# tsbertalan/openmg

Measured on AMD Instinct MI355X. Metric: V-cycles/sec, 3-D 7-point Poisson 256^3, higher is better.
Workload: dtype f64

## Files before the change

openmg_amd/csrc/plane.hip:

```cpp
#include <algorithm>
#include <array>
#include <atomic>
#include <cmath>
#include <cstring>
#include <map>
#include <mutex>
#include <thread>
#include <type_traits>

#include "common.h"
#include "peer_wait.h"
#include "sine_cube16.h"

#if defined(OMG_PLANE_STAMPS) || defined(OMG_PLANE_DBGARGS)
#define OMG_PLANE_DBG_ON 1
#endif

namespace omg {
namespace {

#ifndef PLANE_STORE_AUX
#define PLANE_STORE_AUX 2
#endif
typedef unsigned v2u __attribute__((ext_vector_type(2)));
typedef unsigned v4u __attribute__((ext_vector_type(4)));
typedef int v2i __attribute__((ext_vector_type(2)));

__device__ __forceinline__ double madd(double v, double x, double acc) { return fma(v, x, acc); }
__device__ __forceinline__ float madd(float v, float x, float acc) { return fmaf(v, x, acc); }

template <typename V>
struct P2 {
    V x, y;
};
template <typename V> struct VecOf;
template <> struct VecOf<double> {
    typedef double type __attribute__((ext_vector_type(2)));
    typedef type gtype __attribute__((aligned(8)));
};
template <> struct VecOf<float> {
    typedef float type __attribute__((ext_vector_type(2)));
    typedef type gtype __attribute__((aligned(4)));
};

__device__ __forceinline__ P2<double> bload2(__amdgpu_buffer_rsrc_t rs, int off, double) {
    const v4u q = __builtin_amdgcn_raw_buffer_load_b128(rs, off, 0, 0);
    return {__builtin_bit_cast(double, v2u{q.x, q.y}), __builtin_bit_cast(double, v2u{q.z, q.w})};
}
__device__ __forceinline__ P2<float> bload2(__amdgpu_buffer_rsrc_t rs, int off, float) {
    typedef float v2f __attribute__((ext_vector_type(2)));
    const v2f q = __builtin_bit_cast(v2f, __builtin_amdgcn_raw_buffer_load_b64(rs, off, 0, 0));
    return {q.x, q.y};
}
__device__ __forceinline__ double bload1(__amdgpu_buffer_rsrc_t rs, int off, double) {
    return __builtin_bit_cast(double, __builtin_amdgcn_raw_buffer_load_b64(rs, off, 0, 0));
}
__device__ __forceinline__ float bload1(__amdgpu_buffer_rsrc_t rs, int off, float) {
    return __builtin_bit_cast(float, __builtin_amdgcn_raw_buffer_load_b32(rs, off, 0, 0));
}
template <typename V>
__device__ __forceinline__ P2<V> lds_pair(const V *p) {
    const typename VecOf<V>::type q = *reinterpret_cast<const typename VecOf<V>::type *>(p);
    return {q.x, q.y};
}
template <typename V>
__device__ __forceinline__ void lds_put(V *p, const P2<V> &v) {
    typename VecOf<V>::type q;
    q.x = v.x;
    q.y = v.y;
    *reinterpret_cast<typename VecOf<V>::type *>(p) = q;
}
template <int AUX = PLANE_STORE_AUX>
__device__ __forceinline__ void bstore2(__amdgpu_buffer_rsrc_t rs, int off, const P2<double> &v, bool both) {
    if (both) {
        const v2u lo = __builtin_bit_cast(v2u, v.x), hi = __builtin_bit_cast(v2u, v.y);
        __builtin_amdgcn_raw_buffer_store_b128(v4u{lo.x, lo.y, hi.x, hi.y}, rs, off, 0, AUX);
    } else {
        __builtin_amdgcn_raw_buffer_store_b64(__builtin_bit_cast(v2u, v.x), rs, off, 0, AUX);
    }
}
template <int AUX = 0>
__device__ __forceinline__ void bstore2(__amdgpu_buffer_rsrc_t rs, int off, const P2<float> &v, bool both) {
    if (both) {
        __builtin_amdgcn_raw_buffer_store_b64(v2u{__builtin_bit_cast(unsigned, v.x), __builtin_bit_cast(unsigned, v.y)}, rs, off, 0, AUX);
    } else {
        __builtin_amdgcn_raw_buffer_store_b32(__builtin_bit_cast(unsigned, v.x), rs, off, 0, AUX);
    }
}
template <int AUX>
__device__ __forceinline__ void bstore1(__amdgpu_buffer_rsrc_t rs, int off, double v) {
    __builtin_amdgcn_raw_buffer_store_b64(__builtin_bit_cast(v2u, v), rs, off, 0, AUX);
}
template <int AUX>
__device__ __forceinline__ void bstore1(__amdgpu_buffer_rsrc_t rs, int off, float v) {
    __builtin_amdgcn_raw_buffer_store_b32(__builtin_bit_cast(unsigned, v), rs, off, 0, AUX);
}
constexpr int PEER_PLANES = 3, PEER_CPLANES = 2;
constexpr int PEER_AUX = 1 | 16;
template <typename V>
__device__ __forceinline__ void store2(V *p, const P2<V> &v, bool both) {
    if (both) {
        typename VecOf<V>::gtype q;
        q.x = v.x;
        q.y = v.y;
        *reinterpret_cast<typename VecOf<V>::gtype *>(p) = q;
    } else {
        p[0] = v.x;
    }
}

#ifndef PLANE_LA_BIG
#define PLANE_LA_BIG 1
#endif
#ifndef PLANE_LA
#define PLANE_LA 1
#endif
#ifndef PLANE_WAVE_SYNC
#define PLANE_WAVE_SYNC 1
#endif
constexpr unsigned WAVE_SYNC_SPIN = 1u << 22;
constexpr int OOB = 0x7FFFFFF0;

template <typename V>
struct PlaneKArgs {
    const V *x_old;
    V *x_new;
    const V *b;
    unsigned vec_bytes;
    int nr;
    int hx, ny, nz;
    int z_base, z_end, kv0, kv1, kc_off;
    int TXq, TY, LZ, PX, PY, ntx, nty, ntz;
    int zc_base, zc_stride, zc_len, zc_end, part_slot0;
    int edge_wg0;
    V c0, c1, c2, c3, c4, c5, c6, w;
    V wp;
    int x_zero;
    int fast_div;
    int nxc, nyc, nzc;
    unsigned cvec_bytes, cmap_bytes;
    const int32_t *cmap;
    V *bc, *xc;
    const V *cdiag;
    int first_end;
    const V *ec;
    double *partials;
    V *peer_x[2], *peer_bc[2];
    int peer_shift, peer_cshift;
    const uint32_t *wait_flag[4];
    uint32_t wait_seq[4];
    int fused_wait;
    uint32_t *done, *peer_flag[2];
    uint32_t flag_seq, spin;
    uint32_t *status;
#ifdef OMG_PLANE_STAMPS
    unsigned long long *stamps;
#endif
#ifdef OMG_PLANE_DBG_ON
    int dbg;
#endif
};

template <typename V>
__device__ __forceinline__ V chain_head(const PlaneKArgs<V> &a, V km, V jm, V im) {
    V s = madd(a.c0, km, V(0));
    s = madd(a.c1, jm, s);
    return madd(a.c2, im, s);
}
template <typename V>
__device__ __forceinline__ V chain_tail(const PlaneKArgs<V> &a, V s, V d, V ip, V jp, V kp) {
    s = madd(a.c3, d, s);
    s = madd(a.c4, ip, s);
    s = madd(a.c5, jp, s);
    return madd(a.c6, kp, s);
}

__device__ __forceinline__ double refined_rcp(double d) {
    double r = __builtin_amdgcn_rcp(d);
    double e = fma(-d, r, 1.0);
    r = fma(r, e, r);
    e = fma(-d, r, 1.0);
    return fma(r, e, r);
}
__device__ __forceinline__ float refined_rcp(float) { return 0.0f; }
__device__ __forceinline__ bool plain_numerator(double v) {
    const unsigned e = ((unsigned)__double2hiint(v) >> 20) & 0x7ffu;
    return e - 623u <= 800u || v == 0.0;
}
__device__ __forceinline__ bool plain_numerator(float) { return false; }
template <typename V>
__device__ __forceinline__ void quotients(const V (&n)[4], V c, V r, bool fast, V (&q)[4]) {
    if (sizeof(V) == 8 && fast) {
        bool bad = false;
#pragma unroll
        for (int i = 0; i < 4; ++i) {
            const V q0 = n[i] * r;
            q[i] = madd(madd(-c, q0, n[i]), r, q0);
            bad = bad || !plain_numerator(n[i]);
        }
        if (__builtin_amdgcn_ballot_w64(bad) == 0) return;
    }
#pragma unroll
    for (int i = 0; i < 4; ++i) q[i] = n[i] / c;
}

template <typename V>
struct Inline {
    V imx, ipx, imy, ipy;
};
template <typename V>
__device__ __forceinline__ Inline<V> in_line(int rule, const P2<V> &O, V nb) {
    Inline<V> r;
    r.imx = rule ? O.x : nb;
    r.ipx = rule ? O.y : O.x;
    r.imy = rule ? O.y : O.x;
    r.ipy = rule ? nb : O.y;
    return r;
}

__device__ __forceinline__ void peer_done(uint32_t *done, uint32_t n_wg, uint32_t *const (&flag)[2], uint32_t seq) {
    __builtin_amdgcn_fence(__ATOMIC_RELEASE, "workgroup");
    __syncthreads();
    if (threadIdx.x == 0) {
        const uint32_t before = __hip_atomic_fetch_add(done, 1u, __ATOMIC_RELAXED, __HIP_MEMORY_SCOPE_AGENT);
        if (before == n_wg - 1) {
            __hip_atomic_store(done, 0u, __ATOMIC_RELAXED, __HIP_MEMORY_SCOPE_AGENT);
            for (int i = 0; i < 2; ++i)
                if (flag[i]) __hip_atomic_store(flag[i], seq, __ATOMIC_RELAXED, __HIP_MEMORY_SCOPE_SYSTEM);
        }
    }
}
__global__ void plane_wait_kernel(const uint32_t *f0, const uint32_t *f1, const uint32_t *f2, const uint32_t *f3,
                                  uint32_t s0, uint32_t s1, uint32_t s2, uint32_t s3, uint32_t *status, uint32_t spin) {
    if (threadIdx.x == 0) {
        peer_wait(f0, s0, status, spin);
        peer_wait(f1, s1, status, spin);
        peer_wait(f2, s2, status, spin);
        peer_wait(f3, s3, status, spin);
    }
}

template <typename V, int MODE, bool NORM, bool XZ, int LA, bool PEER = false, int MAXT = 512, bool FIRST = false, bool SWEEP = true, bool MIRROR = false>
__global__ __launch_bounds__(MAXT) void plane_kernel(const PlaneKArgs<V> a) {
    static_assert(!MIRROR || (MODE == 1 && !PEER && !FIRST && !XZ), "mirrored march: up passes of whole grids");
#ifdef OMG_PLANE_STAMPS
    const unsigned long long st_entry = __builtin_amdgcn_s_memtime();
#endif
    extern __shared__ __attribute__((aligned(16))) unsigned char plane_smem[];
    V *const lds = reinterpret_cast<V *>(plane_smem);
    __shared__ double s_red[8];
    __shared__ int s_step[8];
    if (threadIdx.x < 8) s_step[threadIdx.x] = 0;

    const int PX = a.PX, PY = a.PY;
    const int S = 2 * PX + 4;
    const int BUF = (2 * PY + 2) * S;
    const int t = int(threadIdx.x);
    const bool live = t < PX * PY;
    const int px = live ? t % PX : 0, py = live ? t / PX : 0;
    int L = int(blockIdx.x);
    int nwg = int(gridDim.x);
    const bool edge_wg = !PEER && a.edge_wg0 > 0 && L >= a.edge_wg0;
    if (!PEER && a.edge_wg0 > 0) {
        if (edge_wg) { L -= a.edge_wg0; nwg = 1; }
        else nwg = a.edge_wg0;
    }
    if ((nwg & 7) == 0) L = (L & 7) * (nwg >> 3) + (L >> 3);
    const int nxy = a.ntx * a.nty;
    const int tz = L / nxy, rem = L - tz * nxy;
    const int ty = rem / a.ntx, tx = rem - ty * a.ntx;
    const int z0 = edge_wg ? (tz ? a.z_end - PLANE_EDGE : a.z_base) : a.zc_base + tz * a.zc_stride;
    const int z1 = edge_wg ? z0 + PLANE_EDGE : min(a.zc_end, z0 + a.zc_len);
    const int q = tx * a.TXq + px - 1;
    const int ja = ty * a.TY + 2 * py - 4;
    const bool vx0 = live && q >= 0 && 2 * q < a.hx, vx1 = live && q >= 0 && 2 * q + 1 < a.hx;
    const bool vl[2] = {ja >= 0 && ja < a.ny, ja + 1 >= 0 && ja + 1 < a.ny};
    const bool inner = live && px >= 1 && px <= PX - 2 && py >= 2 && py <= PY - 3;
    const int ps = a.ny * a.hx;
    const int lb[2] = {ja * a.hx + 2 * q, (ja + 1) * a.hx + 2 * q};

    const __amdgpu_buffer_rsrc_t xs = __builtin_amdgcn_make_buffer_rsrc(const_cast<V *>(a.x_old), 0, a.vec_bytes, 0x00020000);
    const __amdgpu_buffer_rsrc_t bs = __builtin_amdgcn_make_buffer_rsrc(const_cast<V *>(a.b), 0, a.vec_bytes, 0x00020000);
    const __amdgpu_buffer_rsrc_t ws = __builtin_amdgcn_make_buffer_rsrc(a.x_new, 0, a.vec_bytes, 0x00020000);
    const __amdgpu_buffer_rsrc_t es = __builtin_amdgcn_make_buffer_rsrc(const_cast<V *>(MODE == 1 ? a.ec : a.cdiag), 0, a.cvec_bytes, 0x00020000);
    const __amdgpu_buffer_rsrc_t ms = __builtin_amdgcn_make_buffer_rsrc(const_cast<int32_t *>(a.cmap), 0, a.cmap_bytes, 0x00020000);

    constexpr int W = int(sizeof(V));
    const bool vcell = vl[0] && vx0;
    V c1a = ja > 0 ? a.c1 : V(0);
    V c5b = ja + 2 < a.ny ? a.c5 : V(0);
    V c2x = q > 0 ? a.c2 : V(0);
    V c4x = 2 * q + 1 < a.hx ? a.c4 : V(0);
    V c4y = 2 * q + 2 < a.hx ? a.c4 : V(0);
    unsigned lbo[2] = {vcell ? unsigned(lb[0] * W) : unsigned(OOB), vcell ? unsigned(lb[1] * W) : unsigned(OOB)};
    unsigned lso[2] = {(vcell && inner) ? unsigned(lb[0] * W) : unsigned(OOB), (vcell && inner) ? unsigned(lb[1] * W) : unsigned(OOB)};
    asm volatile("" : "+v"(c1a), "+v"(c5b), "+v"(c2x), "+v"(c4x), "+v"(c4y));
    asm volatile("" : "+v"(lbo[0]), "+v"(lbo[1]), "+v"(lso[0]), "+v"(lso[1]));
    const bool oddx = (a.hx & 1) != 0;

    auto head = [&](int l, int v, int rule, V km, V jm, V im) -> V {
        V sum = madd(a.c0, km, V(0));
        sum = madd(l == 0 ? c1a : a.c1, jm, sum);
        return madd((v == 0 && rule == 0) ? c2x : a.c2, im, sum);
    };
    auto tail = [&](int l, int v, int rule, V sum, V d, V ip, V jp, V kp) -> V {
        sum = madd(a.c3, d, sum);
        sum = madd(rule == 0 ? a.c4 : (v == 0 ? c4x : c4y), ip, sum);
        sum = madd(l == 1 ? c5b : a.c5, jp, sum);
        return madd(a.c6, kp, sum);
    };

    auto zphys = [&](int k) -> int { return MIRROR ? a.nz - 1 - k : k; };
    auto cplane = [&](int kc) -> int { return MIRROR ? (a.nz / 2 - 1 + a.kc_off) - kc : kc + a.kc_off; };
    auto plane_off = [&](int colour, int k) -> unsigned {
        return (k >= a.kv0 && k < a.kv1) ? unsigned(((colour ? a.nr : 0) + zphys(k) * ps) * W) : unsigned(OOB);
    };
    auto fetch = [&](const __amdgpu_buffer_rsrc_t &rs, int colour, int k, int l) -> P2<V> {
        unsigned po = plane_off(colour, k);
        asm volatile("" : "+s"(po));
        return bload2(rs, int(lbo[l] + po), V(0));
    };
    auto fetch_at = [&](const __amdgpu_buffer_rsrc_t &rs, unsigned po, int l) -> P2<V> { return bload2(rs, int(lbo[l] + po), V(0)); };
    auto fetch_x = [&](int colour, int k, int l) -> P2<V> {
        if (XZ) return {V(0), V(0)};
        return fetch(xs, colour, k, l);
    };
    constexpr int XAUX = sizeof(V) == 8 ? PLANE_STORE_AUX : 0;
    auto put_pair = [&](const __amdgpu_buffer_rsrc_t &rs, unsigned off, const P2<V> &v) {
#ifdef OMG_PLANE_DBG_ON
        if (a.dbg & 1) return;
#endif
        if (oddx) {
            bstore1<XAUX>(rs, int(off), v.x);
            bstore1<XAUX>(rs, int(vx1 ? off + unsigned(W) : unsigned(OOB)), v.y);
        } else {
            bstore2(rs, int(off), v, true);
        }
    };
    const bool vcoarse = vcell && (MODE == 1 || inner);
    const int cbase = (ja >> 1) * a.nxc + 2 * q;
    unsigned cb4 = vcoarse ? unsigned(cbase * 4) : unsigned(OOB);
    unsigned lmx = vcoarse ? 0u : unsigned(OOB), lmy = (vcoarse && vx1) ? 0u : unsigned(OOB);
    asm volatile("" : "+v"(cb4), "+v"(lmx), "+v"(lmy));
    const v2u none = {unsigned(OOB), unsigned(OOB)};
    auto slots_request = [&](int kc, bool want) -> v2u {
        kc = cplane(kc);
        const bool ok = want && a.cmap && kc >= 0 && kc < a.nzc;
        return __builtin_amdgcn_raw_buffer_load_b64(ms, int(cb4 + (ok ? unsigned(kc * a.nyc * a.nxc * 4) : unsigned(OOB))), 0, 0);
    };
    auto slots_commit = [&](const v2u &m, int kc, bool want) -> v2u {
        kc = cplane(kc);
        const bool ok = want && kc >= 0 && kc < a.nzc;
        const unsigned u = ok ? 0u : unsigned(OOB), cn = ok ? unsigned(kc * a.nyc * a.nxc * W) : 0u;
        const unsigned s0_ = a.cmap ? m.x * unsigned(W) : cn + cb4 * unsigned(W / 4), s1_ = a.cmap ? m.y * unsigned(W) : cn + cb4 * unsigned(W / 4) + unsigned(W);
        return v2u{s0_ | lmx | u, s1_ | lmy | u};
    };
    auto coarse_slots = [&](int kc) -> v2u { return slots_commit(slots_request(kc, true), kc, true); };
    auto coarse_vals = [&](const v2u &sl) -> P2<V> { return {bload1(es, int(sl.x), V(0)), bload1(es, int(sl.y), V(0))}; };
    auto prolonged = [&](const P2<V> &x, const P2<V> &e) -> P2<V> {
        return {x.x + madd(a.wp, e.x, V(0)), x.y + madd(a.wp, e.y, V(0))};
    };

    const V rc3 = refined_rcp(a.c3);
    const bool fast = a.fast_div != 0;
    const int row_a = 1 + 2 * py, col = 2 + 2 * px;
    const int idx[2] = {row_a * S + col, (row_a + 1) * S + col};
    for (int i = t; i < 6 * BUF; i += int(blockDim.x)) lds[i] = V(0);
    if (((PEER && a.fused_wait) || edge_wg) && t == 0) {
#pragma unroll
        for (int i = 0; i < 4; ++i) peer_wait(a.wait_flag[i], a.wait_seq[i], a.status, a.spin);
    }
    __syncthreads();
    int pside = 0;
    if (PEER) {
        const bool lo = z0 < a.z_base + 2 * PEER_CPLANES, hi = z1 > a.z_end - 2 * PEER_CPLANES;
        pside = (lo && a.peer_x[0] ? 1 : 0) | (hi && a.peer_x[1] ? 2 : 0) | (lo && a.peer_bc[0] ? 4 : 0) | (hi && a.peer_bc[1] ? 8 : 0);
    }
    auto peer_store = [&](int k, int base, const P2<V> (&v)[2]) {
#pragma unroll
        for (int side = 0; side < 2; ++side) {
            const bool hit = side == 0 ? (pside & 1) && k < z0 + PEER_PLANES && k < a.z_base + PEER_PLANES
                                       : (pside & 2) && k >= z1 - PEER_PLANES && k >= a.z_end - PEER_PLANES;
            if (!hit) continue;
            V *px = a.peer_x[side];
            asm volatile("" : "+s"(px));
            const __amdgpu_buffer_rsrc_t pw = __builtin_amdgcn_make_buffer_rsrc(px ? px : a.x_new, 0, px ? a.vec_bytes : 0u, 0x00020000);
            int sh = side == 0 ? a.peer_shift : -a.peer_shift;
            asm volatile("" : "+s"(sh));
#pragma unroll
            for (int l = 0; l < 2; ++l)
                if (vl[l] && vx0) bstore2<PEER_AUX>(pw, (base + sh + lb[l]) * int(sizeof(V)), v[l], vx1);
        }
    };
    int CO_side = 0;
    const __amdgpu_buffer_rsrc_t bcs = __builtin_amdgcn_make_buffer_rsrc(a.bc, 0, a.bc ? a.cvec_bytes : 0u, 0x00020000);
    auto coarse_store = [&](const v2u &sl, const P2<V> &co, const P2<V> &cx, auto PB) {
        bstore1<0>(bcs, int(sl.x), co.x);
        bstore1<0>(bcs, int(sl.y), co.y);
        if (FIRST && a.xc) {
            const __amdgpu_buffer_rsrc_t xcs = __builtin_amdgcn_make_buffer_rsrc(a.xc, 0, a.cvec_bytes, 0x00020000);
            bstore1<0>(xcs, int(sl.x), cx.x);
            bstore1<0>(xcs, int(sl.y), cx.y);
        }
        if (PEER && decltype(PB)::value) {
#pragma unroll
            for (int side = 0; side < 2; ++side) {
                if (!(CO_side & (1 << side))) continue;
                V *pb = a.peer_bc[side];
                int sh = side == 0 ? a.peer_cshift : -a.peer_cshift;
                asm volatile("" : "+s"(pb), "+s"(sh));
                const __amdgpu_buffer_rsrc_t pwb = __builtin_amdgcn_make_buffer_rsrc(pb, 0, a.cvec_bytes, 0x00020000);
                bstore1<PEER_AUX>(pwb, sl.x < unsigned(OOB) ? int(sl.x) + sh * W : OOB, co.x);
                bstore1<PEER_AUX>(pwb, sl.y < unsigned(OOB) ? int(sl.y) + sh * W : OOB, co.y);
            }
        }
    };

    const P2<V> zero2 = {V(0), V(0)};
    P2<V> XR[3][2], XB[5][2], BR[3][2], BB[2], LXB[LA][2], LXR[LA][2], LBR[LA][2], LBB[LA][2], RB[2];
#pragma unroll
    for (int l = 0; l < 2; ++l) {
#pragma unroll
        for (int p = 0; p < 3; ++p) { XR[p][l] = zero2; BR[p][l] = zero2; }
#pragma unroll
        for (int p = 0; p < 5; ++p) XB[p][l] = zero2;
        BB[l] = zero2;
        RB[l] = zero2;
    }
    P2<V> ACC = zero2;
    P2<V> CO = zero2, CX = zero2;
    v2u SLd = none, SLo = none;
    v2u SLt = {0u, 0u};
    int SLt_kc = -1;
    P2<V> DG = zero2, DGt = zero2;
    P2<V> E0 = zero2, E1n = zero2, Et = zero2;
    v2u SLn = none;
    double sq = 0.0, sqy = 0.0;

    const int s0 = z0 - 2;
    constexpr bool RES = MODE == 0 || NORM;
    {
        P2<V> em = zero2;
        if (MODE == 1) {
            const v2u sl0 = coarse_slots(s0 >> 1), slm = coarse_slots((s0 >> 1) - 1);
            SLt_kc = (s0 >> 1) + 1;
            SLt = slots_request(SLt_kc, true);
            E0 = coarse_vals(sl0);
            em = coarse_vals(slm);
        }
#pragma unroll
        for (int l = 0; l < 2; ++l) {
            XB[0][l] = fetch_x(1, s0, l);
            XB[1][l] = RES ? fetch_x(1, s0 - 1, l) : zero2;
            if (MODE == 1) {
                XB[0][l] = prolonged(XB[0][l], E0);
                XB[1][l] = prolonged(XB[1][l], em);
            }
#pragma unroll
            for (int d = 0; d < LA; ++d) {
                LXB[d][l] = fetch_x(1, s0 + d + 1, l);
                LXR[d][l] = (RES || d > 0) ? fetch_x(0, s0 + d, l) : zero2;
                LBR[d][l] = (RES || d > 0) ? fetch(bs, 0, s0 + d, l) : zero2;
                LBB[d][l] = zero2;
            }
            if (live) lds_put(lds + (0 * 2 + (s0 & 1)) * BUF + idx[l], XB[0][l]);
        }
    }
    __syncthreads();

#ifdef OMG_PLANE_STAMPS
    unsigned long long st_mem = 0, st_cmp = 0, st_bar = 0, st_top = 0, st_B = 0, st_C = 0, st_t = __builtin_amdgcn_s_memtime();
#define PLANE_STAMP(acc) { const unsigned long long now_ = __builtin_amdgcn_s_memtime(); acc += now_ - st_t; st_t = now_; }
#else
#define PLANE_STAMP(acc)
#endif
    static_assert(!(PEER && LA == 2), "the two-step loop has no boundary steps");
#ifndef PLANE_WSYNC_F32
#define PLANE_WSYNC_F32 0
#endif
    constexpr bool WSYNC = PLANE_WAVE_SYNC && (sizeof(V) == 8 || PLANE_WSYNC_F32);
    int n_waves = int(blockDim.x) >> 6;
    asm volatile("" : "+s"(n_waves));
    const int my_wave = t >> 6, reach = (PX + 63) >> 6;
    auto publish = [&](int cnt) {
        __builtin_amdgcn_fence(__ATOMIC_RELEASE, "workgroup");
        if ((t & 63) == 0) __hip_atomic_store(&s_step[my_wave], cnt, __ATOMIC_RELAXED, __HIP_MEMORY_SCOPE_WORKGROUP);
    };
    auto await = [&](int cnt) {
        if ((t & 63) == 0) {
            for (int o = max(0, my_wave - reach); o <= min(n_waves - 1, my_wave + reach); ++o)
                for (unsigned polls = 0; __hip_atomic_load(&s_step[o], __ATOMIC_RELAXED, __HIP_MEMORY_SCOPE_WORKGROUP) < cnt; ++polls) {
                    if (polls >= WAVE_SYNC_SPIN) {
                        if (a.status) __hip_atomic_fetch_or(a.status, 2u, __ATOMIC_RELAXED, __HIP_MEMORY_SCOPE_AGENT);
                        break;
                    }
                    __builtin_amdgcn_s_sleep(1);
                }
        }
        __builtin_amdgcn_fence(__ATOMIC_ACQUIRE, "workgroup");
    };
    auto step = [&](auto PARC, const int s, auto PB) {
        constexpr bool PEER_STEP = PEER && decltype(PB)::value;
        const int par = PARC;
        const int set = LA == 2 ? par : 0;
#pragma unroll
        for (int l = 0; l < 2; ++l) {
            asm volatile("" : "+v"(LXB[set][l].x), "+v"(LXB[set][l].y), "+v"(LXR[set][l].x), "+v"(LXR[set][l].y));
            asm volatile("" : "+v"(LBR[set][l].x), "+v"(LBR[set][l].y), "+v"(LBB[set][l].x), "+v"(LBB[set][l].y));
        }
#ifdef OMG_PLANE_STAMPS
        asm volatile("s_waitcnt vmcnt(0)" ::: "memory");
        PLANE_STAMP(st_mem)
#endif
        if (MODE == 1) {
            E1n.x = par ? Et.x : E1n.x; E1n.y = par ? Et.y : E1n.y;
            const v2u sl = slots_commit(SLt, SLt_kc, true);
            SLn.x = par ? SLn.x : sl.x; SLn.y = par ? SLn.y : sl.y;
        } else {
            const v2u sl = slots_commit(SLt, SLt_kc, true);
            SLd.x = par ? SLd.x : sl.x; SLd.y = par ? SLd.y : sl.y;
            if (FIRST) { DG.x = par ? DGt.x : DG.x; DG.y = par ? DGt.y : DG.y; }
        }
#pragma unroll
        for (int l = 0; l < 2; ++l) {
            XB[4][l] = XB[3][l]; XB[3][l] = XB[2][l]; XB[2][l] = XB[1][l]; XB[1][l] = XB[0][l];
            XR[2][l] = XR[1][l]; XR[1][l] = XR[0][l];
            BR[2][l] = BR[1][l]; BR[1][l] = BR[0][l];
            if (MODE == 1) {
                XB[0][l] = prolonged(LXB[set][l], par ? E1n : E0);
                XR[0][l] = prolonged(LXR[set][l], E0);
            } else {
                XB[0][l] = LXB[set][l];
                XR[0][l] = LXR[set][l];
            }
            BR[0][l] = LBR[set][l];
            BB[l] = LBB[set][l];
        }
        if (PEER_STEP && inner && (((pside & 1) && s < z0 + PEER_PLANES + 2) || ((pside & 2) && s >= z1 - PEER_PLANES + 1))) {
            if (s - 1 >= z0 && s - 1 < z1) peer_store(s - 1, (s - 1) * ps, XR[1]);
            if (s - 2 >= z0 && s - 2 < z1) peer_store(s - 2, a.nr + (s - 2) * ps, XB[3]);
        }
        if (MODE == 1) {
            E0.x = par ? E1n.x : E0.x; E0.y = par ? E1n.y : E0.y;
            SLt_kc = (s >> 1) + 2;
            SLt = slots_request(SLt_kc, par != 0);
            Et = coarse_vals(par ? none : SLn);
        } else {
            SLt_kc = (s - 1) >> 1;
            SLt = slots_request(SLt_kc, par != 0);
            if (FIRST) DGt = coarse_vals((par || !a.cdiag) ? none : SLd);
        }
        {
            unsigned pXB = plane_off(1, s + LA + 1), pR = plane_off(0, s + LA), pBB = plane_off(1, s + LA - 1);
            {
                const bool past = s + LA > z1 + (RES ? 1 : 0);
                const int cfirst = z0 - ((RES && SWEEP) ? 1 : 0), clast = z1 - ((RES && SWEEP) ? 0 : 1);
                if (past) { pXB = unsigned(OOB); pR = unsigned(OOB); }
                if (s + LA - 1 < cfirst || s + LA - 1 > clast) pBB = unsigned(OOB);
            }
            asm volatile("" : "+s"(pXB), "+s"(pR), "+s"(pBB));
#ifdef OMG_PLANE_DBG_ON
            if (a.dbg & 16) {
                if (s + LA + 1 < z0 || s + LA + 1 >= z1) pXB = unsigned(OOB);
                if (s + LA < z0 || s + LA >= z1) pR = unsigned(OOB);
                if (s + LA - 1 < z0 || s + LA - 1 >= z1) pBB = unsigned(OOB);
            }
            if (a.dbg & 4) { pXB = unsigned(OOB); }
            unsigned pR_b = pR;
            if (a.dbg & 4) pR = unsigned(OOB);
            if (a.dbg & 8) { pR_b = unsigned(OOB); pBB = unsigned(OOB); }
#else
            const unsigned pR_b = pR;
#endif
#pragma unroll
            for (int l = 0; l < 2; ++l) {
                LXB[set][l] = XZ ? zero2 : fetch_at(xs, pXB, l);
                LXR[set][l] = XZ ? zero2 : fetch_at(xs, pR, l);
                LBR[set][l] = fetch_at(bs, pR_b, l);
                LBB[set][l] = fetch_at(bs, pBB, l);
            }
        }
        if (MODE == 0 && !par && s - 3 >= z0 && s - 3 < z1) {
#ifdef OMG_PLANE_DBG_ON
            if (!(a.dbg & 2))
#endif
            coarse_store(SLo, CO, CX, PB);
        }

        PLANE_STAMP(st_top)
        if (WSYNC) await(s - s0);
        PLANE_STAMP(st_bar)
#ifdef PLANE_SETPRIO
        __builtin_amdgcn_s_setprio(PLANE_SETPRIO);
#endif
        P2<V> d_jm = zero2, d_jp = zero2;
        V d_nb[2] = {V(0), V(0)};
        P2<V> rb[2] = {zero2, zero2};
        if (live) {
            const V *const E1 = lds + (0 * 2 + par) * BUF;
            const V *const E2 = lds + (1 * 2 + par) * BUF;
            const V *const E3 = lds + (2 * 2 + par) * BUF;
            const bool pvB = s >= a.kv0 && s < a.kv1, pvC = s - 1 >= a.kv0 && s - 1 < a.kv1;
            const bool liveT = s > z0 && s <= z1;
            const bool liveB = RES || (s >= z0 - 1 && s <= z1);
            const bool liveC = SWEEP ? (RES ? s >= z0 : liveT) : liveT;
            if (SWEEP && liveB) {
                const P2<V> jm = lds_pair(E1 + idx[0] - S), jp = lds_pair(E1 + idx[1] + S);
                const P2<V> o0 = XB[1][0], o1 = XB[1][1];
                V num[4], quo[4];
#pragma unroll
                for (int l = 0; l < 2; ++l) {
                    const int rule = (l + par + (MIRROR ? 1 : 0)) & 1;
                    const P2<V> O = l ? o1 : o0, Ojm = l ? o0 : jm, Ojp = l ? jp : o1;
                    const Inline<V> n = in_line(rule, O, E1[idx[l] + (rule ? 2 : -1)]);
                    const P2<V> D = XR[0][l], Bv = BR[0][l], Km = XB[MIRROR ? 0 : 2][l], Kp = XB[MIRROR ? 2 : 0][l];
                    num[2 * l] = Bv.x - tail(l, 0, rule, head(l, 0, rule, Km.x, Ojm.x, n.imx), D.x, n.ipx, Ojp.x, Kp.x);
                    num[2 * l + 1] = Bv.y - tail(l, 1, rule, head(l, 1, rule, Km.y, Ojm.y, n.imy), D.y, n.ipy, Ojp.y, Kp.y);
                }
                quotients(num, a.c3, rc3, fast, quo);
#pragma unroll
                for (int l = 0; l < 2; ++l) {
                    XR[0][l].x = XR[0][l].x + quo[2 * l];
                    XR[0][l].y = XR[0][l].y + quo[2 * l + 1];
                }
                if (!pvB) {
                    asm volatile("" ::: "memory");
                    XR[0][0] = zero2; XR[0][1] = zero2;
                }
            }
            if ((SWEEP || MODE == 1) && s - 1 >= z0 && s - 1 < z1) {
                const unsigned base = unsigned(zphys(s - 1) * ps * W);
#pragma unroll
                for (int l = 0; l < 2; ++l) put_pair(ws, lso[l] + base, XR[1][l]);
            }
            PLANE_STAMP(st_B)
            if (liveC) {
                const P2<V> jm = lds_pair(E2 + idx[0] - S), jp = lds_pair(E2 + idx[1] + S);
                const P2<V> o0 = XR[1][0], o1 = XR[1][1];
                V num[4], quo[4], hd[4];
                Inline<V> nl[2];
                P2<V> Jp[2];
#pragma unroll
                for (int l = 0; l < 2; ++l) {
                    const int rule = (l + par + (MIRROR ? 1 : 0)) & 1;
                    const P2<V> O = l ? o1 : o0, Ojm = l ? o0 : jm, Ojp = l ? jp : o1;
                    nl[l] = in_line(rule, O, E2[idx[l] + (rule ? 2 : -1)]);
                    Jp[l] = Ojp;
                    const P2<V> D = XB[2][l], Bv = BB[l], Km = XR[MIRROR ? 0 : 2][l], Kp = XR[MIRROR ? 2 : 0][l];
                    hd[2 * l] = head(l, 0, rule, Km.x, Ojm.x, nl[l].imx);
                    hd[2 * l + 1] = head(l, 1, rule, Km.y, Ojm.y, nl[l].imy);
                    num[2 * l] = Bv.x - tail(l, 0, rule, hd[2 * l], D.x, nl[l].ipx, Ojp.x, Kp.x);
                    num[2 * l + 1] = Bv.y - tail(l, 1, rule, hd[2 * l + 1], D.y, nl[l].ipy, Ojp.y, Kp.y);
                }
                if (SWEEP) quotients(num, a.c3, rc3, fast, quo);
#pragma unroll
                for (int l = 0; l < 2; ++l) {
                    if (!SWEEP) {
                        rb[l].x = num[2 * l];
                        rb[l].y = num[2 * l + 1];
                        continue;
                    }
                    XB[2][l].x = XB[2][l].x + quo[2 * l];
                    XB[2][l].y = XB[2][l].y + quo[2 * l + 1];
                }
                if (SWEEP && RES && liveT) {
#pragma unroll
                    for (int l = 0; l < 2; ++l) {
                        const int rule = (l + par + (MIRROR ? 1 : 0)) & 1;
                        const P2<V> Bv = BB[l], Kp = XR[MIRROR ? 2 : 0][l];
                        rb[l].x = Bv.x - tail(l, 0, rule, hd[2 * l], XB[2][l].x, nl[l].ipx, Jp[l].x, Kp.x);
                        rb[l].y = Bv.y - tail(l, 1, rule, hd[2 * l + 1], XB[2][l].y, nl[l].ipy, Jp[l].y, Kp.y);
                    }
                }
                if (!pvC) {
                    asm volatile("" ::: "memory");
                    XB[2][0] = zero2; XB[2][1] = zero2;
                    rb[0] = zero2; rb[1] = zero2;
                }
            }
            if ((SWEEP || MODE == 1) && s - 2 >= z0 && s - 2 < z1) {
                const unsigned base = unsigned((a.nr + zphys(s - 2) * ps) * W);
#pragma unroll
                for (int l = 0; l < 2; ++l) put_pair(ws, lso[l] + base, XB[3][l]);
            }
            PLANE_STAMP(st_C)
#pragma unroll
            for (int l = 0; l < 2; ++l) d_nb[l] = E3[idx[l] + (((l + par + (MIRROR ? 1 : 0)) & 1) ? 2 : -1)];
            d_jm = lds_pair(E3 + idx[0] - S);
            d_jp = lds_pair(E3 + idx[1] + S);
            V *const W1 = lds + (0 * 2 + (par ^ 1)) * BUF;
            V *const W2 = lds + (1 * 2 + (par ^ 1)) * BUF;
            V *const W3 = lds + (2 * 2 + (par ^ 1)) * BUF;
#pragma unroll
            for (int l = 0; l < 2; ++l) {
                lds_put(W1 + idx[l], XB[0][l]);
                lds_put(W2 + idx[l], XR[0][l]);
                lds_put(W3 + idx[l], XB[2][l]);
            }
        }
        PLANE_STAMP(st_cmp)
#ifdef PLANE_SETPRIO
        __builtin_amdgcn_s_setprio(0);
#endif
        if (WSYNC) publish(s - s0 + 1);
        else __syncthreads();
        PLANE_STAMP(st_bar)
        if (live) {
            P2<V> rr[2] = {zero2, zero2};
            if (RES && s >= z0 + 2) {
                const P2<V> jm = d_jm, jp = d_jp;
                const P2<V> o0 = XB[3][0], o1 = XB[3][1];
#pragma unroll
                for (int l = 0; l < 2; ++l) {
                    const int rule = (l + par + (MIRROR ? 1 : 0)) & 1;
                    const P2<V> O = l ? o1 : o0, Ojm = l ? o0 : jm, Ojp = l ? jp : o1;
                    const Inline<V> n = in_line(rule, O, d_nb[l]);
                    const P2<V> D = XR[2][l], Bv = BR[2][l], Km = XB[MIRROR ? 2 : 4][l], Kp = XB[MIRROR ? 4 : 2][l];
                    rr[l].x = Bv.x - tail(l, 0, rule, head(l, 0, rule, Km.x, Ojm.x, n.imx), D.x, n.ipx, Ojp.x, Kp.x);
                    rr[l].y = Bv.y - tail(l, 1, rule, head(l, 1, rule, Km.y, Ojm.y, n.imy), D.y, n.ipy, Ojp.y, Kp.y);
                }
            }
            if (MODE == 0) {
                if (!par) {
                    ACC.x = madd(a.w, rr[0].x, V(0)); ACC.y = madd(a.w, rr[0].y, V(0));
                    ACC.x = madd(a.w, RB[0].x, ACC.x); ACC.y = madd(a.w, RB[0].y, ACC.y);
                    ACC.x = madd(a.w, RB[1].x, ACC.x); ACC.y = madd(a.w, RB[1].y, ACC.y);
                    ACC.x = madd(a.w, rr[1].x, ACC.x); ACC.y = madd(a.w, rr[1].y, ACC.y);
                } else {
                    ACC.x = madd(a.w, RB[0].x, ACC.x); ACC.y = madd(a.w, RB[0].y, ACC.y);
                    ACC.x = madd(a.w, rr[0].x, ACC.x); ACC.y = madd(a.w, rr[0].y, ACC.y);
                    ACC.x = madd(a.w, rr[1].x, ACC.x); ACC.y = madd(a.w, rr[1].y, ACC.y);
                    ACC.x = madd(a.w, RB[1].x, ACC.x); ACC.y = madd(a.w, RB[1].y, ACC.y);
                    if (s - 2 >= z0 && s - 2 < z1) {
                        CO = ACC;
                        SLo = SLd;
                        if (PEER) CO_side = (((pside & 4) && s - 2 < z0 + 2 * PEER_CPLANES && s - 2 < a.z_base + 2 * PEER_CPLANES) ? 1 : 0) |
                                            (((pside & 8) && s - 2 >= z1 - 2 * PEER_CPLANES && s - 2 >= a.z_end - 2 * PEER_CPLANES) ? 2 : 0);
                        if (FIRST) {
                            CX.x = (a.cdiag && SLd.x < unsigned(a.first_end) * unsigned(W)) ? V(0) + (ACC.x - V(0)) / DG.x : V(0);
                            CX.y = (a.cdiag && SLd.y < unsigned(a.first_end) * unsigned(W)) ? V(0) + (ACC.y - V(0)) / DG.y : V(0);
                        }
                    }
                }
                RB[0] = rb[0];
                RB[1] = rb[1];
            }
            if (NORM) {
                if (s - 1 >= z0 && s - 1 < z1) {
#pragma unroll
                    for (int l = 0; l < 2; ++l) {
                        sq = fma(double(rb[l].x), double(rb[l].x), sq);
                        sqy = fma(double(rb[l].y), double(rb[l].y), sqy);
                    }
                }
                if (s - 2 >= z0 && s - 2 < z1) {
#pragma unroll
                    for (int l = 0; l < 2; ++l) {
                        sq = fma(double(rr[l].x), double(rr[l].x), sq);
                        sqy = fma(double(rr[l].y), double(rr[l].y), sqy);
                    }
                }
            }
        }
        PLANE_STAMP(st_cmp)
    };
    if (LA == 2) {
        for (int s = s0; s <= z1 + 1; s += 2) {
            step(std::integral_constant<int, 0>(), s, std::false_type());
            step(std::integral_constant<int, 1>(), s + 1, std::false_type());
        }
    } else {
        constexpr bool PAIRS = !FIRST;
        if (PAIRS) {
            for (int s = s0; s <= z1 + 1; s += 2) {
                step(std::integral_constant<int, 0>(), s, std::integral_constant<bool, PEER>());
                step(std::integral_constant<int, 1>(), s + 1, std::integral_constant<bool, PEER>());
            }
        } else {
            for (int s = s0; s <= z1 + 1; ++s) step(s & 1, s, std::integral_constant<bool, PEER>());
        }
    }
#ifdef OMG_PLANE_STAMPS
    if ((t & 63) == 0) {
        unsigned long long *o = a.stamps + (size_t(blockIdx.x) * 8 + (t >> 6)) * 8;
        o[0] = st_mem; o[1] = st_cmp; o[2] = st_bar; o[3] = unsigned(z1 + 2 - s0); o[4] = st_top; o[5] = st_B; o[6] = st_C;
        o[7] = __builtin_amdgcn_s_memtime() - st_entry;
    }
#endif
    if (MODE == 0 && z1 > z0) coarse_store(SLo, CO, CX, std::true_type());
    if (NORM) {
        sq = (inner && vcell) ? sq + (vx1 ? sqy : 0.0) : 0.0;
#pragma unroll
        for (int off = 32; off > 0; off >>= 1) sq += __shfl_down(sq, off, 64);
        if ((t & 63) == 0) s_red[t >> 6] = sq;
        __syncthreads();
        if (t == 0) {
            double tot = 0.0;
            for (int wv = 0; wv < int(blockDim.x) >> 6; ++wv) tot += s_red[wv];
            a.partials[a.part_slot0 + int(blockIdx.x)] = tot;
        }
    }
    if (PEER) peer_done(a.done, gridDim.x, a.peer_flag, a.flag_seq);
}

template <typename V>
struct PlaneSpmvArgs {
    const V *x;
    V *y;
    unsigned vec_bytes;
    int nr, hx, ny, nz, hq;
    V c0, c1, c2, c3, c4, c5, c6;
};
template <typename V>
__global__ __launch_bounds__(256) void plane_spmv_kernel(const PlaneSpmvArgs<V> a) {
    const int64_t t = int64_t(blockIdx.x) * 256 + threadIdx.x;
    const int64_t per_colour = int64_t(a.hq) * a.ny * a.nz;
    if (t >= 2 * per_colour) return;
    const int colour = t >= per_colour ? 1 : 0;
    const int64_t u = t - colour * per_colour;
    const int q = int(u % a.hq);
    const int line = int(u / a.hq), j = line % a.ny, k = line / a.ny;
    const int h = 2 * q;
    const bool two = h + 1 < a.hx;
    const int p = (j + k) & 1;
    const __amdgpu_buffer_rsrc_t xs = __builtin_amdgcn_make_buffer_rsrc(const_cast<V *>(a.x), 0, a.vec_bytes, 0x00020000);
    const __amdgpu_buffer_rsrc_t ys = __builtin_amdgcn_make_buffer_rsrc(a.y, 0, a.vec_bytes, 0x00020000);
    const int same = colour ? a.nr : 0, other = colour ? 0 : a.nr;
    const int lb = line * a.hx + h;
    const int ps = a.ny * a.hx;
    auto pair_at = [&](int base, bool ok) -> P2<V> {
        P2<V> r = bload2(xs, ok ? (base + lb) * int(sizeof(V)) : OOB, V(0));
        if (!two) r.y = V(0);
        return r;
    };
    const P2<V> D = pair_at(same, true);
    const P2<V> Km = pair_at(other - ps, k > 0), Kp = pair_at(other + ps, k + 1 < a.nz);
    const P2<V> Jm = pair_at(other - a.hx, j > 0), Jp = pair_at(other + a.hx, j + 1 < a.ny);
    const P2<V> O = pair_at(other, true);
    const int rule = colour ? 1 - p : p;
    const int nbh = rule ? h + 2 : h - 1;
    const V nb = bload1(xs, (nbh >= 0 && nbh < a.hx) ? (other + line * a.hx + nbh) * int(sizeof(V)) : OOB, V(0));
    const Inline<V> n = in_line(rule, O, nb);
    PlaneKArgs<V> c;
    c.c0 = a.c0; c.c1 = a.c1; c.c2 = a.c2; c.c3 = a.c3; c.c4 = a.c4; c.c5 = a.c5; c.c6 = a.c6;
    P2<V> out;
    out.x = chain_tail(c, chain_head(c, Km.x, Jm.x, n.imx), D.x, n.ipx, Jp.x, Kp.x);
    out.y = chain_tail(c, chain_head(c, Km.y, Jm.y, n.imy), D.y, n.ipy, Jp.y, Kp.y);
    bstore2<0>(ys, (same + lb) * int(sizeof(V)), out, two);
}

template <typename V>
struct PlaneSpmvMarchArgs {
    PlaneSpmvArgs<V> s;
    int qt, lpw, njg, nqt, lz;
};
template <typename V>
__global__ __launch_bounds__(512) void plane_spmv_march_kernel(const PlaneSpmvMarchArgs<V> m) {
    const PlaneSpmvArgs<V> &a = m.s;
    int L = int(blockIdx.x);
    const int nwg = int(gridDim.x);
    if ((nwg & 7) == 0) L = (L & 7) * (nwg >> 3) + (L >> 3);
    const int per_chunk = m.njg * m.nqt;
    const int zc = L / per_chunk, rem = L - zc * per_chunk;
    const int jg = rem / m.nqt, qg = rem - jg * m.nqt;
    const int t = int(threadIdx.x);
    const int q = qg * m.qt + t % m.qt, j = jg * m.lpw + t / m.qt;
    const bool live = t < m.qt * m.lpw && q < a.hq && j < a.ny;
    const int h = 2 * q;
    const bool two = h + 1 < a.hx;
    const __amdgpu_buffer_rsrc_t xs = __builtin_amdgcn_make_buffer_rsrc(const_cast<V *>(a.x), 0, a.vec_bytes, 0x00020000);
    const __amdgpu_buffer_rsrc_t ys = __builtin_amdgcn_make_buffer_rsrc(a.y, 0, a.vec_bytes, 0x00020000);
    const int ps = a.ny * a.hx;
    const int W = int(sizeof(V));
    const int lb = j * a.hx + h;
    auto pair_at = [&](int colour, int k, int dj) -> P2<V> {
        const bool ok = live && k >= 0 && k < a.nz && j + dj >= 0 && j + dj < a.ny;
        P2<V> r = bload2(xs, ok ? ((colour ? a.nr : 0) + k * ps + lb + dj * a.hx) * W : OOB, V(0));
        if (!two) r.y = V(0);
        return r;
    };
    auto one_at = [&](int colour, int k, int hh) -> V {
        const bool ok = live && hh >= 0 && hh < a.hx;
        return bload1(xs, ok ? ((colour ? a.nr : 0) + k * ps + j * a.hx + hh) * W : OOB, V(0));
    };
    PlaneKArgs<V> c;
    c.c0 = a.c0; c.c1 = a.c1; c.c2 = a.c2; c.c3 = a.c3; c.c4 = a.c4; c.c5 = a.c5; c.c6 = a.c6;
    const int z0 = zc * m.lz, z1 = min(a.nz, z0 + m.lz);
    P2<V> X[2][3];
#pragma unroll
    for (int col = 0; col < 2; ++col) { X[col][0] = pair_at(col, z0 - 1, 0); X[col][1] = pair_at(col, z0, 0); }
    for (int k = z0; k < z1; ++k) {
        P2<V> Jm[2], Jp[2];
        V nb[2];
        const int p = (j + k) & 1;
#pragma unroll
        for (int col = 0; col < 2; ++col) {
            X[col][2] = pair_at(col, k + 1, 0);
            Jm[col] = pair_at(col, k, -1);
            Jp[col] = pair_at(col, k, 1);
            const int rule = col ? p : 1 - p;
            nb[col] = one_at(col, k, rule ? h + 2 : h - 1);
        }
#pragma unroll
        for (int col = 0; col < 2; ++col) {
            const int o = 1 - col;
            const int rule = col ? 1 - p : p;
            const Inline<V> n = in_line(rule, X[o][1], nb[o]);
            P2<V> out;
            out.x = chain_tail(c, chain_head(c, X[o][0].x, Jm[o].x, n.imx), X[col][1].x, n.ipx, Jp[o].x, X[o][2].x);
            out.y = chain_tail(c, chain_head(c, X[o][0].y, Jm[o].y, n.imy), X[col][1].y, n.ipy, Jp[o].y, X[o][2].y);
            if (live) bstore2<0>(ys, ((col ? a.nr : 0) + k * ps + lb) * W, out, two);
        }
#pragma unroll
        for (int col = 0; col < 2; ++col) { X[col][0] = X[col][1]; X[col][1] = X[col][2]; }
    }
}

template <typename V>
struct BlockKArgs {
    const V *x_old;
    V *x_new;
    const V *b;
    int nx, ny, nz, nr;
    int nbx, nby;
    V c0, c1, c2, c3, c4, c5, c6, w;
    V wp;
    int fast_div;
    int nxc, nyc;
    const int32_t *cmap;
    V *bc;
    const V *ec;
};
// ... 1426 lines not shown
```

Measured before the change: 3923.

## Replace two warm-up march steps with a dedicated prologue for non-peer plane kernels

For non-peer launches, the march now starts at z0 instead of z0-2. A specialized entry block issues the boundary-plane loads together, runs the two stage-B updates the first two steps used to perform, and seeds the LDS images and lookahead registers. The wave-sync counters start at -1 so the prologue can publish step 0. This removes two full pipelined steps and their barriers from the start of each plane kernel, at the cost of a longer, more complex prologue that raises register pressure and adds correctness risk at the plane boundaries.

Result: no change. 3950, median of 2 (+0.7%).

```diff
diff --git a/openmg_amd/csrc/plane.hip b/openmg_amd/csrc/plane.hip
--- a/openmg_amd/csrc/plane.hip
+++ b/openmg_amd/csrc/plane.hip
@@ -250,7 +250,8 @@
     V *const lds = reinterpret_cast<V *>(plane_smem);
     __shared__ double s_red[8];
     __shared__ int s_step[8];
-    if (threadIdx.x < 8) s_step[threadIdx.x] = 0;
+    constexpr bool ENTRY = !PEER;
+    if (threadIdx.x < 8) s_step[threadIdx.x] = ENTRY ? -1 : 0;
 
     const int PX = a.PX, PY = a.PY;
     const int S = 2 * PX + 4;
@@ -437,9 +438,9 @@
     v2u SLn = none;
     double sq = 0.0, sqy = 0.0;
 
-    const int s0 = z0 - 2;
+    const int s0 = ENTRY ? z0 : z0 - 2;
     constexpr bool RES = MODE == 0 || NORM;
-    {
+    if constexpr (!ENTRY) {
         P2<V> em = zero2;
         if (MODE == 1) {
             const v2u sl0 = coarse_slots(s0 >> 1), slm = coarse_slots((s0 >> 1) - 1);
@@ -465,8 +466,8 @@
             }
             if (live) lds_put(lds + (0 * 2 + (s0 & 1)) * BUF + idx[l], XB[0][l]);
         }
-    }
-    __syncthreads();
+        __syncthreads();
+    }
 
 #ifdef OMG_PLANE_STAMPS
     unsigned long long st_mem = 0, st_cmp = 0, st_bar = 0, st_top = 0, st_B = 0, st_C = 0, st_t = __builtin_amdgcn_s_memtime();
@@ -499,6 +500,130 @@
         }
         __builtin_amdgcn_fence(__ATOMIC_ACQUIRE, "workgroup");
     };
+    auto stage_b = [&](const int par, const V *const img, P2<V> (&R)[2], const P2<V> (&Bv_)[2], const P2<V> (&Kb)[2],
+                       const P2<V> (&O_)[2], const P2<V> (&Ka)[2], const bool pv, auto ZIMG) {
+        if (!SWEEP) return;
+        constexpr bool ZI = decltype(ZIMG)::value;
+        const P2<V> jm = ZI ? zero2 : lds_pair(img + idx[0] - S), jp = ZI ? zero2 : lds_pair(img + idx[1] + S);
+        const P2<V> o0 = O_[0], o1 = O_[1];
+        V num[4], quo[4];
+#pragma unroll
+        for (int l = 0; l < 2; ++l) {
+            const int rule = (l + par + (MIRROR ? 1 : 0)) & 1;
+            const P2<V> O = l ? o1 : o0, Ojm = l ? o0 : jm, Ojp = l ? jp : o1;
+            const Inline<V> n = in_line(rule, O, ZI ? V(0) : img[idx[l] + (rule ? 2 : -1)]);
+            const P2<V> D = R[l], Bv = Bv_[l], Km = MIRROR ? Ka[l] : Kb[l], Kp = MIRROR ? Kb[l] : Ka[l];
+            num[2 * l] = Bv.x - tail(l, 0, rule, head(l, 0, rule, Km.x, Ojm.x, n.imx), D.x, n.ipx, Ojp.x, Kp.x);
+            num[2 * l + 1] = Bv.y - tail(l, 1, rule, head(l, 1, rule, Km.y, Ojm.y, n.imy), D.y, n.ipy, Ojp.y, Kp.y);
+        }
+        quotients(num, a.c3, rc3, fast, quo);
+#pragma unroll
+        for (int l = 0; l < 2; ++l) {
+            R[l].x = R[l].x + quo[2 * l];
+            R[l].y = R[l].y + quo[2 * l + 1];
+        }
+        if (!pv) {
+            asm volatile("" ::: "memory");
+            R[0] = zero2; R[1] = zero2;
+        }
+    };
+    if constexpr (ENTRY) {
+        const int kc0 = z0 >> 1;
+        v2u q0 = none, q1 = none, q2 = none;
+        if (MODE == 1) {
+            q1 = slots_request(kc0 - 1, true);
+            q0 = slots_request(kc0, true);
+            q2 = slots_request(kc0 - 2, RES);
+            SLt_kc = kc0 + 1;
+        } else {
+            SLt_kc = (z0 - 2) >> 1;
+        }
+        SLt = slots_request(SLt_kc, true);
+        V *const I_b0 = lds + (0 * 2 + 0) * BUF, *const I_b1 = lds + (0 * 2 + 1) * BUF;
+        V *const I_r0 = lds + (1 * 2 + 0) * BUF, *const I_n0 = lds + (2 * 2 + 0) * BUF;
+#pragma unroll
+        for (int l = 0; l < 2; ++l) {
+            XB[1][l] = fetch_x(1, z0 - 1, l);
+            XB[2][l] = fetch_x(1, z0 - 2, l);
+        }
+        P2<V> em1 = zero2, em2 = zero2;
+        if (MODE == 1) {
+            em1 = coarse_vals(slots_commit(q1, kc0 - 1, true));
+            E0 = coarse_vals(slots_commit(q0, kc0, true));
+            em2 = coarse_vals(slots_commit(q2, kc0 - 2, RES));
+        }
+#pragma unroll
+        for (int l = 0; l < 2; ++l) {
+            XB[3][l] = RES ? fetch_x(1, z0 - 3, l) : zero2;
+            XR[1][l] = RES ? fetch_x(0, z0 - 2, l) : zero2;
+            BR[1][l] = RES ? fetch(bs, 0, z0 - 2, l) : zero2;
+        }
+#pragma unroll
+        for (int l = 0; l < 2; ++l) {
+            XB[0][l] = fetch_x(1, z0, l);
+            XR[0][l] = fetch_x(0, z0 - 1, l);
+            BR[0][l] = fetch(bs, 0, z0 - 1, l);
+        }
+#pragma unroll
+        for (int l = 0; l < 2; ++l) {
+#pragma unroll
+            for (int d = 0; d < LA; ++d) {
+                unsigned pXB = plane_off(1, z0 + d + 1), pR = plane_off(0, z0 + d), pBB = plane_off(1, z0 + d - 1);
+                const int cfirst = z0 - ((RES && SWEEP) ? 1 : 0), clast = z1 - ((RES && SWEEP) ? 0 : 1);
+                if (z0 + d > z1 + (RES ? 1 : 0)) { pXB = unsigned(OOB); pR = unsigned(OOB); }
+                if (z0 + d - 1 < cfirst || z0 + d - 1 > clast) pBB = unsigned(OOB);
+                asm volatile("" : "+s"(pXB), "+s"(pR), "+s"(pBB));
+                LXB[d][l] = XZ ? zero2 : fetch_at(xs, pXB, l);
+                LXR[d][l] = XZ ? zero2 : fetch_at(xs, pR, l);
+                LBR[d][l] = fetch_at(bs, pR, l);
+                LBB[d][l] = fetch_at(bs, pBB, l);
+            }
+        }
+        if (MODE == 1) {
+#pragma unroll
+            for (int l = 0; l < 2; ++l) {
+                XB[1][l] = prolonged(XB[1][l], em1);
+                XB[2][l] = prolonged(XB[2][l], em1);
+            }
+        }
+        if (!XZ && live) {
+#pragma unroll
+            for (int l = 0; l < 2; ++l) {
+                lds_put(I_b1 + idx[l], XB[1][l]);
+                lds_put(I_n0 + idx[l], XB[2][l]);
+            }
+        }
+        __builtin_amdgcn_fence(__ATOMIC_RELEASE, "workgroup", "local");
+        __builtin_amdgcn_s_barrier();
+        __builtin_amdgcn_fence(__ATOMIC_ACQUIRE, "workgroup", "local");
+        if (live) {
+            if (RES) {
+                if (MODE == 1) {
+#pragma unroll
+                    for (int l = 0; l < 2; ++l) {
+                        XB[3][l] = prolonged(XB[3][l], em2);
+                        XR[1][l] = prolonged(XR[1][l], em1);
+                    }
+                }
+                stage_b(0, I_n0, XR[1], BR[1], XB[3], XB[2], XB[1], z0 - 2 >= a.kv0 && z0 - 2 < a.kv1, std::integral_constant<bool, XZ>());
+            }
+            if (MODE == 1) {
+#pragma unroll
+                for (int l = 0; l < 2; ++l) {
+                    XB[0][l] = prolonged(XB[0][l], E0);
+                    XR[0][l] = prolonged(XR[0][l], em1);
+                }
+            }
+            stage_b(1, I_b1, XR[0], BR[0], XB[2], XB[1], XB[0], z0 - 1 >= a.kv0 && z0 - 1 < a.kv1, std::integral_constant<bool, XZ>());
+#pragma unroll
+            for (int l = 0; l < 2; ++l) {
+                if (!XZ) lds_put(I_b0 + idx[l], XB[0][l]);
+                lds_put(I_r0 + idx[l], XR[0][l]);
+            }
+        }
+        if (WSYNC) publish(0);
+        else __syncthreads();
+    }
     auto step = [&](auto PARC, const int s, auto PB) {
         constexpr bool PEER_STEP = PEER && decltype(PB)::value;
         const int par = PARC;
@@ -604,30 +729,7 @@
             const bool liveT = s > z0 && s <= z1;
             const bool liveB = RES || (s >= z0 - 1 && s <= z1);
             const bool liveC = SWEEP ? (RES ? s >= z0 : liveT) : liveT;
-            if (SWEEP && liveB) {
-                const P2<V> jm = lds_pair(E1 + idx[0] - S), jp = lds_pair(E1 + idx[1] + S);
-                const P2<V> o0 = XB[1][0], o1 = XB[1][1];
-                V num[4], quo[4];
-#pragma unroll
-                for (int l = 0; l < 2; ++l) {
-                    const int rule = (l + par + (MIRROR ? 1 : 0)) & 1;
-                    const P2<V> O = l ? o1 : o0, Ojm = l ? o0 : jm, Ojp = l ? jp : o1;
-                    const Inline<V> n = in_line(rule, O, E1[idx[l] + (rule ? 2 : -1)]);
-                    const P2<V> D = XR[0][l], Bv = BR[0][l], Km = XB[MIRROR ? 0 : 2][l], Kp = XB[MIRROR ? 2 : 0][l];
-                    num[2 * l] = Bv.x - tail(l, 0, rule, head(l, 0, rule, Km.x, Ojm.x, n.imx), D.x, n.ipx, Ojp.x, Kp.x);
-                    num[2 * l + 1] = Bv.y - tail(l, 1, rule, head(l, 1, rule, Km.y, Ojm.y, n.imy), D.y, n.ipy, Ojp.y, Kp.y);
-                }
-                quotients(num, a.c3, rc3, fast, quo);
-#pragma unroll
-                for (int l = 0; l < 2; ++l) {
-                    XR[0][l].x = XR[0][l].x + quo[2 * l];
-                    XR[0][l].y = XR[0][l].y + quo[2 * l + 1];
-                }
-                if (!pvB) {
-                    asm volatile("" ::: "memory");
-                    XR[0][0] = zero2; XR[0][1] = zero2;
-                }
-            }
+            if (SWEEP && liveB) stage_b(par, E1, XR[0], BR[0], XB[2], XB[1], XB[0], pvB, std::false_type());
             if ((SWEEP || MODE == 1) && s - 1 >= z0 && s - 1 < z1) {
                 const unsigned base = unsigned(zphys(s - 1) * ps * W);
 #pragma unroll
```
